# patrickltobing/shallow-wavenet

Measured on AMD Instinct MI355X. Metric: decoded samples/sec (22.05 kHz Laplacian AR decode, whole job), higher is better.
Workload: dtype f32

## Files before the change

include/swn_hip.h:

```cpp
#ifndef SWN_HIP_H
#define SWN_HIP_H

#include <stddef.h>
#include <stdint.h>

#ifdef __cplusplus
extern "C" {
#endif

#define SWN_ABI_VERSION 3

#define SWN_PRECISION_FP32 0
#define SWN_PRECISION_BF16 1

#define SWN_KIND_LAPLACE 0
#define SWN_KIND_SOFTMAX 1

#define SWN_OK            0
#define SWN_E_BADDESC    -1
#define SWN_E_BADARG     -2
#define SWN_E_LAUNCH     -3
#define SWN_E_UNSUPPORTED -4
#define SWN_E_NODEVICE   -5

// ... 47 lines not shown
    int32_t n_new;
    int32_t f0, f1;
    int32_t flags;
    int32_t reserved[2];
} swn_frontend_pool_entry;
#define SWN_FRONTEND_POOL_MAX_ENTRIES 64
#define SWN_FRONTEND_FINAL 1
size_t swn_frontend_pool_work_floats(const swn_net_desc* d, const swn_frontend_pool_entry* entries_host, int n_entries);
int    swn_frontend_pool(const swn_net_desc* d, const float* packed_dev, const swn_frontend_pool_entry* entries_host,
                         int n_entries, float* work_dev, void* stream);

#define SWN_POOL_MAX_MODELS 16
size_t swn_frontend_pool_models_work_floats(const swn_net_desc* d, const swn_frontend_pool_entry* entries_host,
                                            const int32_t* model_of_entry_host, int n_entries, int n_models);
int    swn_frontend_pool_models(const swn_net_desc* d, const float* const* models_host, int n_models,
                                const int32_t* model_of_entry_host, const swn_frontend_pool_entry* entries_host,
                                int n_entries, float* work_dev, void* stream);

typedef struct swn_decode_io {
    const float* noise_dev;
    const void*  forced_dev;
    const void*  seed_dev;
    float*       noise_out_dev;
    uint64_t     rng_seed;
    uint32_t     rng_utt0;
    uint32_t     reserved;
    const uint32_t* rng_utt_ids_dev;
} swn_decode_io;
size_t swn_decode_state_floats(const swn_net_desc* d, int batch);
int    swn_decode(const swn_net_desc* d, const float* packed_dev, const float* cond_dev,
                  int batch, int n_frames, int n_steps, const swn_decode_io* io,
                  float* state_dev, void* out_dev, float* heads_dev,
                  int variant, void* stream);

#define SWN_CHUNK_BEGIN 1
int    swn_decode_resolve_variant(const swn_net_desc* d, int batch, int variant);
size_t swn_decode_session_floats(const swn_net_desc* d, int batch, int variant);
int    swn_decode_chunk(const swn_net_desc* d, const float* packed_dev, const float* cond_dev, int batch, int n_frames,
                        int step0, int n_steps, int flags, const swn_decode_io* io, float* session_dev,
                        void* out_dev, float* heads_dev, int variant, void* stream);

typedef struct swn_decode_pool_entry {
    const float* cond_dev;
    int32_t n_frames;
    int32_t slot;
    int32_t step0;
    int32_t n_steps;
    int32_t flags;
    int32_t reserved;
} swn_decode_pool_entry;
#define SWN_DECODE_POOL_MAX_ENTRIES 64
int    swn_decode_pool_chunk(const swn_net_desc* d, const float* packed_dev, int capacity,
                             const swn_decode_pool_entry* entries_host, int n_entries,
                             const swn_decode_io* io, float* session_dev,
                             void* out_dev, float* heads_dev, int variant, void* stream);
int    swn_decode_pool_chunk_models(const swn_net_desc* d, const float* const* models_host, int n_models,
                                    const int32_t* model_of_entry_host, int capacity,
                                    const swn_decode_pool_entry* entries_host, int n_entries,
                                    const swn_decode_io* io, float* session_dev,
                                    void* out_dev, float* heads_dev, int variant, void* stream);

size_t swn_decode_w16_bytes(const swn_net_desc* d);
int    swn_pack_decode_w16(const swn_net_desc* d, const float* packed_dev, void* w16_dev, void* stream);
int    swn_decode_w16(const swn_net_desc* d, const float* packed_dev, const float* cond_dev,
                      int batch, int n_frames, int n_steps, const swn_decode_io* io,
                      float* state_dev, void* out_dev, float* heads_dev, int variant, const void* w16_dev, void* stream);
// ... 291 lines not shown
```

shallow_wavenet_amd/_lib.py:

```python
from __future__ import annotations

import ctypes
import os
import subprocess
import threading
from ctypes import POINTER, c_char_p, c_float, c_int, c_int32, c_int64, c_size_t, c_void_p

from .config import NetConfig

_HERE = os.path.dirname(os.path.abspath(__file__))
LIB_PATH = os.environ.get("SWN_HIP_LIB", os.path.join(_HERE, "libswn_hip.so"))
CSRC = os.path.join(_HERE, "csrc")

_lock = threading.Lock()
_lib = None


class NetDesc(ctypes.Structure):
    _fields_ = [(n, c_int32) for n in (
        "kind", "n_aux", "hid_chn", "skip_chn", "aux_kernel_size", "aux_dilation_size",
        "dilation_depth", "dilation_repeat", "kernel_size", "upsampling_factor", "seg", "lpc",
        "n_quantize", "wav_conv_flag", "audio_in_flag", "aux_conv2d_flag")]


# ... 84 lines not shown
                   aux_kernel_size=cfg.aux_kernel_size, aux_dilation_size=cfg.aux_dilation_size,
                   dilation_depth=cfg.dilation_depth, dilation_repeat=cfg.dilation_repeat,
                   kernel_size=cfg.kernel_size, upsampling_factor=cfg.upsampling_factor,
                   seg=1 if soft else cfg.seg, lpc=0 if soft else cfg.lpc,
                   n_quantize=cfg.n_quantize if soft else 0,
                   wav_conv_flag=int(cfg.wav_conv_flag), audio_in_flag=int(cfg.audio_in_flag and soft),
                   aux_conv2d_flag=int(cfg.aux_conv2d_flag and not soft))


SIGNATURES = {
    "swn_abi_version": (c_int, []),
    "swn_strerror": (c_char_p, [c_int]),
    "swn_last_error_detail": (c_char_p, []),
    "swn_device_count": (c_int, []),
    "swn_receptive_field": (c_int, [POINTER(NetDesc)]),
    "swn_num_tensors": (c_int, [POINTER(NetDesc)]),
    "swn_packed_floats": (c_size_t, [POINTER(NetDesc)]),
    "swn_layout_offsets": (c_int, [POINTER(NetDesc), POINTER(c_size_t), c_int]),
    "swn_pack_params": (c_int, [POINTER(NetDesc), POINTER(c_void_p), c_int, c_void_p, c_size_t]),
    "swn_pack_params_device": (c_int, [POINTER(NetDesc), POINTER(c_void_p), c_int, c_void_p, c_size_t, c_void_p]),
    "swn_frontend_conv_lds_bytes": (c_size_t, [POINTER(NetDesc), c_int]),
    "swn_frontend_work_floats": (c_size_t, [POINTER(NetDesc), c_int, c_int]),
    "swn_cond_floats": (c_size_t, [POINTER(NetDesc), c_int, c_int]),
    "swn_frontend": (c_int, [POINTER(NetDesc), c_void_p, c_void_p, c_int, c_int, c_void_p, c_void_p, c_void_p]),
    "swn_frontend_pool_work_floats": (c_size_t, [POINTER(NetDesc), POINTER(FrontendPoolEntry), c_int]),
    "swn_frontend_pool": (c_int, [POINTER(NetDesc), c_void_p, POINTER(FrontendPoolEntry), c_int, c_void_p, c_void_p]),
    "swn_frontend_pool_models_work_floats": (c_size_t, [POINTER(NetDesc), POINTER(FrontendPoolEntry), POINTER(c_int32), c_int,
                                                        c_int]),
    "swn_frontend_pool_models": (c_int, [POINTER(NetDesc), POINTER(c_void_p), c_int, POINTER(c_int32),
                                         POINTER(FrontendPoolEntry), c_int, c_void_p, c_void_p]),
    "swn_decode_state_floats": (c_size_t, [POINTER(NetDesc), c_int]),
    "swn_decode": (c_int, [POINTER(NetDesc), c_void_p, c_void_p, c_int, c_int, c_int, POINTER(DecodeIO),
                           c_void_p, c_void_p, c_void_p, c_int, c_void_p]),
    "swn_decode_resolve_variant": (c_int, [POINTER(NetDesc), c_int, c_int]),
    "swn_decode_session_floats": (c_size_t, [POINTER(NetDesc), c_int, c_int]),
    "swn_decode_chunk": (c_int, [POINTER(NetDesc), c_void_p, c_void_p, c_int, c_int, c_int, c_int, c_int, POINTER(DecodeIO),
                                 c_void_p, c_void_p, c_void_p, c_int, c_void_p]),
    "swn_decode_pool_chunk": (c_int, [POINTER(NetDesc), c_void_p, c_int, POINTER(DecodePoolEntry), c_int, POINTER(DecodeIO),
                                      c_void_p, c_void_p, c_void_p, c_int, c_void_p]),
    "swn_decode_pool_chunk_models": (c_int, [POINTER(NetDesc), POINTER(c_void_p), c_int, POINTER(c_int32), c_int,
                                             POINTER(DecodePoolEntry), c_int, POINTER(DecodeIO), c_void_p, c_void_p, c_void_p,
                                             c_int, c_void_p]),
    "swn_decode_pool_wide_table_bytes": (c_size_t, [c_int]),
    "swn_decode_pool_chunk_wide": (c_int, [POINTER(NetDesc), POINTER(c_void_p), c_int, POINTER(c_int32), c_int,
                                           POINTER(DecodePoolEntry), c_int, POINTER(DecodeIO), c_void_p, c_void_p, c_void_p,
                                           c_int, POINTER(c_void_p), c_int, c_void_p, c_void_p]),
    "swn_e4m3_table": (c_int, [c_void_p, c_float, c_void_p]),
    "swn_decode_stepped_prologue_iterations": (c_int, [POINTER(NetDesc)]),
    "swn_decode_pool_stepped_chunk": (c_int, [POINTER(NetDesc), c_void_p, c_int, POINTER(DecodeSteppedPoolEntry), c_int,
                                              POINTER(DecodeIO), c_void_p, c_void_p, c_void_p, c_void_p]),
    "swn_decode_stepped_pool_plan": (c_int, [POINTER(c_int32), POINTER(c_int32), c_int, c_int, c_int, POINTER(c_int32),
                                             POINTER(c_int32)]),
    "swn_decode_pool_stepped_chunk_models": (c_int, [POINTER(NetDesc), POINTER(c_void_p), c_int, POINTER(c_int32), c_int,
                                                     POINTER(DecodeSteppedPoolEntry), c_int, POINTER(DecodeIO), c_void_p,
                                                     c_void_p, c_void_p, c_void_p]),
    "swn_decode_stepped_prologue_work_floats": (c_size_t, [POINTER(NetDesc), c_int]),
    "swn_decode_stepped_prologue": (c_int, [POINTER(NetDesc), c_void_p, POINTER(c_void_p), c_int, POINTER(c_int32), c_int,
                                            POINTER(DecodeSteppedPrologueEntry), c_int, POINTER(DecodeIO), c_void_p, c_void_p,
                                            c_void_p]),
    "swn_postfilter_state_doubles": (c_size_t, [c_int, c_int, c_int]),
    "swn_postfilter_chunk": (c_int, [c_int, ctypes.c_double, c_int, c_void_p, c_int, c_void_p, c_void_p, c_void_p, c_int,
                                     POINTER(PostfilterEntry), c_int, c_void_p]),
    "swn_forward_work_floats": (c_size_t, [POINTER(NetDesc), c_int, c_int]),
    "swn_forward": (c_int, [POINTER(NetDesc), c_void_p, c_void_p, c_void_p, c_int, c_int, c_void_p,
                            c_void_p, c_void_p, c_void_p]),
    "swn_bf16_weight_bytes": (c_size_t, [POINTER(NetDesc)]),
# ... 150 lines not shown
```

shallow_wavenet_amd/csrc/swn_decode_bl6w.hip:

```cpp
#include <type_traits>
#include "swn_decode_bl6_common.hpp"
#include "swn_decode_internal.hpp"

#ifndef SWN_RES_SLICE
#define SWN_RES_SLICE 0
#endif
#ifndef SWN_ROTATE
#define SWN_ROTATE 1
#endif
#ifndef SWN_HANDOFF
#define SWN_HANDOFF 0
#endif
#ifndef SWN_OLDER2_MERGED
#define SWN_OLDER2_MERGED 1
#endif
#ifndef SWN_EARLY_ROWS
#define SWN_EARLY_ROWS 1
#endif
#ifndef SWN_LEAD
#define SWN_LEAD 1
#endif
#ifndef SWN_RINGX
#define SWN_RINGX 1
#endif
#ifdef SWN_STAMP
#define SWN_TDEF_PARAM , unsigned long long& tdef
#define SWN_TDEF_ARG(k) , td[k]
#else
#define SWN_TDEF_PARAM
#define SWN_TDEF_ARG(k)
#endif

namespace {

using namespace swn_bl6;

constexpr int NG = 256;
constexpr int S = 128;
constexpr int O1 = 128;

template <int LPC_, bool EXT_>
struct Tw {
    static constexpr int LPC = LPC_;
    static constexpr bool EXT = EXT_;
    using Ext = Tw<LPC_, true>;
    static constexpr bool NEWFORM = !EXT_ && LPC_ == 0;
    static constexpr int LEAD = NEWFORM ? SWN_LEAD : 0;
    static constexpr bool RINGX = NEWFORM && SWN_RINGX;
    static constexpr int NO = 2 + LPC_;
    static constexpr int WN = cmax(1, LPC_) + 1;
    static constexpr int ring_len(int l) { return pow2ceil((1 << l) + 1); }
    static constexpr int ring_off(int l) { int o = 0; for (int i = 0; i < l; ++i) o += ring_len(i) * H; return o; }
    static constexpr int PF = L * 2 * H;
    static constexpr int NZC = 64, NZB = 4;
    static constexpr int o_ring = 0;
    static constexpr int o_hcat = o_ring + ring_off(L);
    static constexpr int o_gp = o_hcat + L * H;
    static constexpr int o_bx = o_gp + 2 * PF;
    static constexpr int o_bd = o_bx + L * 2 * H;
    static constexpr int o_old = o_bd + L * 2 * H;
    static constexpr int o_wup = o_old + 2 * L * 2 * H;
    static constexpr int o_skip = o_wup + 256;
    static constexpr int o_p2 = o_skip + S;
    static constexpr int o_tnz = o_p2 + 4 * NO;
    static constexpr int o_cz = o_tnz + r4(NZB * NZC);
    static constexpr int o_w2 = o_cz + 5 * H;
    static constexpr int o_bias = o_w2 + NO * S + r4(NO);
    static constexpr int o_w1 = o_bias + S + O1;
    static constexpr int o_wl = o_w1 + 8 * O1 * 16;
    static constexpr int o_h0w = o_wl + 8 * NG * 4;
    static constexpr int o_ho = o_h0w + 3 * H;
    static constexpr int HO = 4, NHO = 128;
    static constexpr int o_end = o_ho + (NEWFORM && (SWN_HANDOFF & 1) && SWN_ROTATE ? NHO * HO : 0);
    static constexpr size_t lds_bytes = (size_t)o_end * sizeof(float);
    static constexpr int sess_old = ring_off(L);
    static constexpr int sess_win = sess_old + 2 * L * 2 * H;
    static constexpr int sess_floats = sess_win + r4(WN);
};

__device__ __forceinline__ float sum_quads(float v) {
    v += dpp_f<0x124>(v);
    v += dpp_f<0x128>(v);
    float w = v;
    asm("s_nop 1\n\tv_permlane16_swap_b32 %0, %1" : "+v"(v), "+v"(w));
    v += w;
    w = v;
    asm("s_nop 1\n\tv_permlane32_swap_b32 %0, %1" : "+v"(v), "+v"(w));
    return v + w;
}
__device__ __forceinline__ float quad_sum_by_parity(float own, float other) {
    float s = own + dpp_f<0xB1>(other);
    s += dpp_f<0x4E>(s);
    return s;
}
struct NoWork { __device__ __forceinline__ void operator()() const {} };
template <class T, int LAYER, int NQ = 2, class BEHIND = NoWork>
__device__ __forceinline__ void layer_a(float* lds, const float (&w)[2][16], const int q, const float wj, const int pb, const int po,
                                        const int ta, const float* xr, BEHIND&& behind = NoWork{}) {
    constexpr bool ROT = !std::is_same<typename std::decay<BEHIND>::type, NoWork>::value;
    const int o = ta >> 2, p = ta & 3, pr = p & 1;
    const float e_old = lds[T::o_old + po + LAYER * 2 * H + pr * H + o];
    const float g_gp = lds[T::o_gp + pb + LAYER * 2 * H + pr * H + o], g_bx = lds[T::o_bx + LAYER * 2 * H + pr * H + o];
    const float e_hp = xr[o];
    static_assert(NQ >= 0 && NQ <= 4, "early quads");
    float4 xq[4];
    if constexpr (ROT) {
#pragma unroll
        for (int m = 0; m < NQ; ++m) xq[m] = *reinterpret_cast<const float4*>(xr + 16 * p + 4 * m);
        __builtin_amdgcn_sched_barrier(0);
        behind();
        __builtin_amdgcn_sched_barrier(0);
    }
    const float e_gx = fmaf(wj, g_gp, g_bx);
    float az = 0.f, ac = 0.f;
#pragma unroll
    for (int m = 0; m < 4; ++m) {
        float4 x;
        if (ROT && m < NQ) x = xq[m];
        else x = *reinterpret_cast<const float4*>(xr + 16 * p + 4 * m);
        az = fmaf(w[0][4 * m], x.x, az); ac = fmaf(w[1][4 * m], x.x, ac);
        az = fmaf(w[0][4 * m + 1], x.y, az); ac = fmaf(w[1][4 * m + 1], x.y, ac);
        az = fmaf(w[0][4 * m + 2], x.z, az); ac = fmaf(w[1][4 * m + 2], x.z, ac);
        az = fmaf(w[0][4 * m + 3], x.w, az); ac = fmaf(w[1][4 * m + 3], x.w, ac);
    }
    const float sq = quad_sum_by_parity(pr ? ac : az, pr ? az : ac);
    __builtin_amdgcn_sched_barrier(0);
    if (p < 2) {
        const float sa = sq + e_old;
        const float v = e_gx * sa;
#ifdef SWN_DIAG_PLAINEXP
        const float e = __builtin_amdgcn_exp2f((p == 0 ? -v : -2.f * fminf(fabsf(v), 64.f)) * 1.44269504f);
        const float r = __builtin_amdgcn_rcpf(1.f + e);
#else
        const float e = exp_c(p == 0 ? -v : -2.f * fminf(fabsf(v), 64.f));
        const float r = rcp_c(1.f + e);
#endif
        const float res = p == 0 ? r : copysignf((1.f - e) * r, v);
        const float c = dpp_f<0xF5>(res);
        if (p == 0) {
            const float hn = (1.f - res) * c + res * e_hp;
            if (LAYER + 1 < L) {
                constexpr int R2 = T::ring_len(LAYER + 1 < L ? LAYER + 1 : LAYER);
                lds[T::o_ring + T::ring_off(LAYER + 1 < L ? LAYER + 1 : LAYER) + (q & (R2 - 1)) * H + o] = hn;
            }
            if (!T::RINGX || LAYER + 1 >= L) lds[T::o_hcat + LAYER * H + o] = hn;
        }
    }
    __builtin_amdgcn_sched_barrier(0);
}

template <class T, int LAYER, int MB = 4>
__device__ __forceinline__ void older_sum(const float* lds, const float (&w)[2][16], const int qn, const int tb, float& az, float& ac) {
    constexpr int dil = 1 << LAYER;
    constexpr int R = T::ring_len(LAYER);
    const int p = tb & 3;
    const float* ring = lds + T::o_ring + T::ring_off(LAYER);
    az = 0.f; ac = 0.f;
#pragma unroll
    for (int m = 0; m < 4; ++m) {
        const float4 x = *reinterpret_cast<const float4*>(ring + ((qn - dil) & (R - 1)) * H + 16 * p + 4 * m);
        float4 w0, w1;
        if (LAYER < L - 1) {
            w0 = make_float4(w[0][4 * m], w[0][4 * m + 1], w[0][4 * m + 2], w[0][4 * m + 3]);
            w1 = make_float4(w[1][4 * m], w[1][4 * m + 1], w[1][4 * m + 2], w[1][4 * m + 3]);
        } else {
            w0 = *reinterpret_cast<const float4*>(lds + T::o_wl + (m * NG + tb) * 4);
            w1 = *reinterpret_cast<const float4*>(lds + T::o_wl + ((4 + m) * NG + tb) * 4);
        }
        az = fmaf(w0.x, x.x, az); ac = fmaf(w1.x, x.x, ac);
        az = fmaf(w0.y, x.y, az); ac = fmaf(w1.y, x.y, ac);
        az = fmaf(w0.z, x.z, az); ac = fmaf(w1.z, x.z, ac);
        az = fmaf(w0.w, x.w, az); ac = fmaf(w1.w, x.w, ac);
        if (MB < 4 && m % MB == MB - 1) __builtin_amdgcn_sched_barrier(0);
    }
    az = sum4(az); ac = sum4(ac);
}
template <class T, int LAYER>
__device__ __forceinline__ void older_store(float* lds, const int qn, const int tb, const float az, const float ac) {
    const int o = tb >> 2, p = tb & 3, pr = p & 1;
    lds[T::o_old + (qn & 1) * (L * 2 * H) + LAYER * 2 * H + pr * H + o] = (p == 0 ? az : ac) + lds[T::o_bd + LAYER * 2 * H + pr * H + o];
}
// ... 144 lines not shown
        }
        __builtin_amdgcn_sched_barrier(0);
    }
    asm volatile("" : "+v"(sacc[0]), "+v"(sacc[1]));
}
template <class T>
__device__ __forceinline__ void skip_last_b(float* lds, const float4 (&wsl)[8], const float (&sacc)[2], const int tb) {
    const int r = tb >> 2, hp = tb & 3;
    float part[2][4];
#pragma unroll
    for (int mm = 0; mm < 4; ++mm) {
        const float4 x = *reinterpret_cast<const float4*>(lds + T::o_hcat + (L - 1) * H + 16 * mm + 4 * hp);
#pragma unroll
        for (int ps = 0; ps < 2; ++ps) {
            const float4 w = wsl[ps * 4 + mm];
            part[ps][mm] = fmaf(w.w, x.w, fmaf(w.z, x.z, fmaf(w.y, x.y, w.x * x.x)));
        }
    }
    float s[2];
#pragma unroll
    for (int ps = 0; ps < 2; ++ps) s[ps] = sacc[ps] + ((part[ps][0] + part[ps][1]) + (part[ps][2] + part[ps][3]));
    const float t0 = s[0] + dpp_f<0xB1>(s[0]), t1 = s[1] + dpp_f<0xB1>(s[1]);
    const float v = (hp < 2 ? t0 : t1) + dpp_f<0x4E>(hp < 2 ? t1 : t0);
    if ((hp & 1) == 0) lds[T::o_skip + r + 32 * hp] = fmaxf(v, 0.f);
}

template <bool MOVE2> using OlderMergedT = typename std::conditional<MOVE2, Layers<2, 3, 4>, Layers<3, 4>>::type;
template <bool MOVE2> using OlderOut1T = typename std::conditional<MOVE2, Layers<0, 1>, Layers<0, 1, 2>>::type;
template <int E> struct Out1Split;
template <> struct Out1Split<2> { using Early = Layers<0, 1>; using Late = Layers<>; };
template <> struct Out1Split<1> { using Early = Layers<0>; using Late = Layers<1>; };
template <> struct Out1Split<0> { using Early = Layers<>; using Late = Layers<0, 1>; };

template <class T, bool GA, bool STREAM, bool POOL = false>
__device__ __forceinline__ void decode_body(const Bl6Args& a, float* lds) {
    constexpr bool EXT = T::EXT;
    static_assert(!STREAM || EXT, "streamed chunks run the extended mode");
    constexpr bool grpA = GA;
    const int tid = threadIdx.x, b = POOL ? 0 : blockIdx.x;
    __builtin_assume(GA ? tid < NG : tid >= NG);
    const int tg = tid & (NG - 1);
    const float* __restrict__ P = a.P;
    const int U = a.U;
    const int s0 = STREAM ? a.step0 : 0;
    const bool resume = STREAM && a.resume;
    const int fb0 = STREAM ? s0 / U : 0;

    for (int e = tid; e < T::o_end; e += NT) lds[e] = 0.f;
    __syncthreads();
    for (int e = tid; e < L * 2 * H; e += NT) {
        lds[T::o_bx + e] = P[a.y.bx + e];
        const float bd = P[a.y.bd + e];
        lds[T::o_bd + e] = bd;
        lds[T::o_old + e] = bd;
    }
    for (int e = tid; e < U; e += NT) lds[T::o_wup + e] = P[a.y.wup + e];
    for (int e = tid; e < H; e += NT) lds[T::o_cz + e] = P[a.y.cb + e];
    for (int e = tid; e < S; e += NT) lds[T::o_bias + e] = P[a.y.bsk + e];
    for (int e = tid; e < O1; e += NT) lds[T::o_bias + S + e] = P[a.y.b1 + e];
    for (int e = tid; e < 2 * H; e += NT) { lds[T::o_cz + H + e] = P[a.y.cv + e]; lds[T::o_cz + 3 * H + e] = P[a.y.cc + e]; }
    for (int e = tid; e < T::NO * S; e += NT) lds[T::o_w2 + e] = P[a.y.w2 + (size_t)(e / S) * r4(S) + (e % S)];
    for (int e = tid; e < T::NO; e += NT) lds[T::o_w2 + T::NO * S + e] = P[a.y.b2 + e];
    for (int e = tid; e < 8 * O1 * 16; e += NT) lds[T::o_w1 + e] = P[a.y.w12 + e];
    const __amdgpu_buffer_rsrc_t condr =
        make_rsrc(a.cond + (size_t)b * a.Tf * a.N, (unsigned)((size_t)a.Tf * a.N * sizeof(float)));
    auto load_frame = [&](int fr) {
        float* dst = lds + T::o_gp + (fr & 1) * T::PF;
#pragma unroll
        for (int it = 0; it < (T::PF / 4 + NT - 1) / NT; ++it) {
            const int e4 = it * NT + tid;
            if (e4 < T::PF / 4)
                *reinterpret_cast<float4*>(dst + 4 * e4) =
                    buf_ld4(condr, (unsigned)tid * 16u, (unsigned)(fr * a.N * 4 + it * NT * 16));
        }
    };
    for (int fr = fb0; fr < fb0 + 2 && fr < a.Tf; ++fr) load_frame(fr);
    constexpr int NWR = grpA ? L : L - 1;
    float wreg[NWR][2][16];
    {
        const int o = tg >> 2, p = tg & 3, k = grpA ? 1 : 0;
#pragma unroll
        for (int l = 0; l < L; ++l)
#pragma unroll
            for (int r = 0; r < 2; ++r) {
                const float4* src = reinterpret_cast<const float4*>(P + a.y.wd + (((size_t)l * 2 * H + o + r * H) * 2 + k) * H + 16 * p);
#pragma unroll
                for (int v = 0; v < 4; ++v) {
                    const float4 t = src[v];
                    if (l == L - 1 && !grpA) {
                        *reinterpret_cast<float4*>(lds + T::o_wl + ((r * 4 + v) * NG + tg) * 4) = t;
                    } else {
                        float (&wr)[16] = wreg[l < NWR ? l : 0][r];
                        wr[4 * v] = t.x; wr[4 * v + 1] = t.y; wr[4 * v + 2] = t.z; wr[4 * v + 3] = t.w;
                    }
                }
            }
    }
    __syncthreads();
    const float* sess_b = STREAM ? a.sess + (size_t)b * T::sess_floats : nullptr;
    int tcp = tid;
    asm volatile("" : "+v"(tcp));
    if (resume) {
        for (int e = tcp; e < T::ring_off(L); e += NT) lds[T::o_ring + e] = sess_b[e];
        for (int e = tcp; e < 2 * L * 2 * H; e += NT) lds[T::o_old + e] = sess_b[T::sess_old + e];
        __syncthreads();
    }

    int fb = fb0, tb0 = fb0 * U;
    const int n_pro = RF;
    auto cond_taps = [&](int q, float& wj, int& pb) {
        const int t0 = q - RF;
        const int tlo = t0 < 0 ? 0 : t0;
        if (tlo >= tb0 + U) {
            fb += 1; tb0 += U;
            if (fb + 1 < a.Tf) load_frame(fb + 1);
        }
        int rel = tlo - tb0;
        int fsel = fb;
// ... 71 lines not shown
                const float sg = (e > 0.f) ? 1.f : ((e < 0.f) ? -1.f : 0.f);
                lds[T::o_tnz + (c & (T::NZB - 1)) * T::NZC + k] = sg * log1pf(-2.f * fabsf(e));
            }
            if (!EXT) noise_load(c + 1);
        }
    };
    if (!EXT && NZG && tn >= 64 && tn < 128) noise_load(0);
    noise_chunk(0);
    noise_chunk(1);

    const __amdgpu_buffer_rsrc_t wsk2 = make_rsrc(P + a.y.wsk2, (unsigned)(L * S * 64 * sizeof(float)));
    constexpr bool NEWFORM = T::NEWFORM;
    constexpr int RES = (grpA || !NEWFORM) ? -1 : SWN_RES_SLICE;
    static_assert(RES == -1 || RES == 0 || RES == L - 1, "the first or the last slice");
    constexpr int LEADB = RES == 0 ? T::LEAD : 0;
    static_assert(LEADB == 0 || LEADB == 1 || LEADB == 2 || LEADB == 4, "one load, a quarter or a half of a slice");
    float4 wres[8];
    if constexpr (RES == 0) skip_issue_b<0>(wsk2, wres, tg, 0u);
    if constexpr (RES == L - 1) skip_issue_b<L - 1>(wsk2, wres, tg, 0u);

#ifdef SWN_STAMP
    unsigned long long tw[9] = {0, 0, 0, 0, 0, 0, 0, 0, 0}, tv[6] = {0, 0, 0, 0, 0, 0}, td[5] = {0, 0, 0, 0, 0}, tstep = 0, tlast = 0, tbeg = 0;
#define SWN_BAR(k) { tw[k] += __builtin_amdgcn_s_memtime() - tlast; lds_barrier(); tlast = __builtin_amdgcn_s_memtime(); }
#define SWN_WAIT_STAMP(k) { asm volatile("" :: "v"(wsl[0].x)); tv[k] += __builtin_amdgcn_s_memtime() - tlast; }
#define SWN_PRE(k) { tw[k] += __builtin_amdgcn_s_memtime() - tlast; asm volatile("s_waitcnt lgkmcnt(0)" ::: "memory"); }
#define SWN_BAR_KEEP(k, N) { lds_barrier_keep<N>(); tlast = __builtin_amdgcn_s_memtime(); }
#else
#define SWN_BAR(k) lds_barrier();
#define SWN_WAIT_STAMP(k)
#define SWN_PRE(k)
#define SWN_BAR_KEEP(k, N) lds_barrier_keep<N>();
#endif
#define SWN_PHASE_WORK(LAYER, GEN, X0)                                                                                \
    if constexpr (grpA) layer_a<T, LAYER>(lds, wreg[LAYER], q, wj, pb, po, tg,                                         \
                                          LAYER == 0 ? (X0) : lds + T::o_ring + T::ring_off(LAYER) +                   \
                                                                  (q & (T::ring_len(LAYER) - 1)) * H);                 \
    else {                                                                                                             \
        if (GEN) {    \
                      \
                      \
                      \
            if (LAYER == 0) { if (RES != 0) skip_issue_b<0>(wsk2, wsl, tg, step0); }                                   \
                      \
            else if (LAYER == 1 && RES == 0)                                                                           \
                skip_roll_b<T, 1, !NOSTREAM, LEADB, LEADB, true>(lds, wsk2, wres, wsl, sacc, tg, step0, q SWN_TDEF_ARG(0)); \
            else { SWN_WAIT_STAMP(LAYER > 0 ? LAYER - 1 : 0)                                                           \
                   skip_roll_b<T, (LAYER > 0 ? LAYER : 1), !(LAYER == L - 1 && RES == L - 1) && !NOSTREAM,             \
                               (LAYER >= 2 ? LEADB : 0), (LAYER < L - 1 ? LEADB : 0)>(lds, wsk2, wsl, wsl, sacc, tg, step0, q \
                                                                                      SWN_TDEF_ARG(LAYER > 0 ? LAYER - 1 : 0)); } \
            __builtin_amdgcn_sched_barrier(0);                                                                         \
        }                                                                                                              \
        if (!(GEN)) older_b<T, LAYER>(lds, wreg[LAYER < NWR ? LAYER : 0], q + 1, tg);                                  \
        else if (LAYER == 0) older_bn<T>(OlderMerged{}, lds, wreg, q + 1, tg);                                         \
        __builtin_amdgcn_sched_barrier(0);                                                                             \
    }
#define SWN_PHASE(LAYER, GEN, X0) SWN_PHASE_WORK(LAYER, GEN, X0) if (GEN) { SWN_BAR(LAYER) } else lds_barrier();

#pragma unroll 1
    for (int q = resume ? n_pro : 0; q < n_pro; ++q) {
        float wj; int pb;
        float4 wsl[8]; float sacc[2]; const unsigned step0 = 0;
        cond_taps(q, wj, pb);
        const int po = (q & 1) * (L * 2 * H);
        input_seed(q);
        lds_barrier();
        const float* x0 = lds + T::o_ring + (q & 1) * H;
        SWN_PHASE(0, false, x0) SWN_PHASE(1, false, x0) SWN_PHASE(2, false, x0) SWN_PHASE(3, false, x0)
        SWN_PHASE(4, false, x0) SWN_PHASE(5, false, x0)
        (void)wsl; (void)sacc; (void)step0;
    }

    int rel_c = s0 - fb0 * U;
    bool fill_c = false;
    float wj_c = 0.f;
    int pb_c = 0, po_c = 0, x0_c = 0;
    auto taps_ahead = [&](int qn) {
        wj_c = lds[T::o_wup + rel_c];
        pb_c = (fb & 1) * T::PF;
        po_c = (qn & 1) * (L * 2 * H);
        x0_c = h0_row(qn);
        asm volatile("" : "+s"(pb_c), "+s"(po_c), "+s"(x0_c));
    };
    auto frame_advance = [&]() {
        rel_c += 1;
        const bool cross = rel_c >= U;
        if (cross) { rel_c = 0; fb += 1; }
        fill_c = cross && fb + 1 < a.Tf;
    };
    if constexpr (grpA) taps_ahead(RF + s0);
    input_gen(x0_c);
#ifdef SWN_STAMP
    tlast = tbeg = __builtin_amdgcn_s_memtime();
#endif
    constexpr bool ROT = SWN_ROTATE && NEWFORM;
    constexpr int ROTQ = 2;
    float sv_p = 0.f, acc_p = 0.f;
    const __amdgpu_buffer_rsrc_t outr =
        make_rsrc(reinterpret_cast<float*>(a.out) + (size_t)b * a.n_steps, (unsigned)((size_t)a.n_steps * sizeof(float)));
    const __amdgpu_buffer_rsrc_t headr =
        make_rsrc(HEADS_ON && a.heads ? a.heads + (size_t)b * a.n_steps * T::NO : nullptr,
                  HEADS_ON && a.heads ? (unsigned)((size_t)a.n_steps * T::NO * sizeof(float)) : 0u);
    auto store_step = [&](const int ip) __attribute__((always_inline)) {
// ... 18 lines not shown
        }
    };
    auto load_frame_b = [&](int fr) {
        if (tg < T::PF / 4)
            *reinterpret_cast<float4*>(lds + T::o_gp + (fr & 1) * T::PF + 4 * tg) =
                buf_ld4(condr, (unsigned)tg * 16u, (unsigned)(fr * a.N * 4));
    };
    auto store_chunk_b = [&](const int c) __attribute__((always_inline)) {
        const int step = c * 64 + tg;
        if (tg < 64 && step < a.n_steps) {
            const float4 v = *reinterpret_cast<const float4*>(lds + T::o_ho + (step & (T::NHO - 1)) * T::HO);
            __builtin_amdgcn_raw_buffer_store_b32(__builtin_bit_cast(unsigned, v.z), outr, (unsigned)tg * 4u, (unsigned)c * 256u, 0);
            using u2 = unsigned __attribute__((ext_vector_type(2)));
            u2 h; h.x = __builtin_bit_cast(unsigned, v.x); h.y = __builtin_bit_cast(unsigned, v.y);
            __builtin_amdgcn_raw_buffer_store_b64(h, headr, (unsigned)tg * 8u, (unsigned)c * 512u, 0);
        }
    };
    auto gen_step = [&](const int i) __attribute__((always_inline)) {
        const int q = RF + s0 + i;
        const float wj = wj_c;
        const int pb = pb_c, po = po_c;
        if constexpr (grpA && !ROT) {
            if (fill_c) load_frame(fb + 1);
        }
        auto behind0 = [&]() __attribute__((always_inline)) {
            if constexpr (NOSIDE) return;
            if constexpr (!HO_NZ) { if ((i & (T::NZC - 1)) == 0) noise_chunk((i >> 6) + 2); }
            if constexpr (!HO_RF) { if (fill_c) load_frame(fb + 1); }
            if constexpr (HO_ST) { if (i > 0) ho_write(i - 1); }
            else { if (i > 0) store_step(i - 1); }
        };
        float4 wsl[8];
        float sacc[2] = {0.f, 0.f};
        if constexpr (!grpA) {
            const float bs0 = lds[T::o_bias + (tg >> 2)], bs1 = lds[T::o_bias + (tg >> 2) + 64];
            if ((tg & 3) == 0) { sacc[0] = bs0; sacc[1] = bs1; }
        }
        unsigned step0 = 0;
        asm volatile("" : "+s"(step0));
        const float* x0 = lds + x0_c;
#ifdef SWN_DIAG_NOSIDE_B
        constexpr bool SIDE_B = false;
#else
        constexpr bool SIDE_B = HOFF && !grpA && !NOSIDE;
#endif
        if constexpr (SIDE_B) {
            __builtin_amdgcn_sched_barrier(0);
            if constexpr (HO_NZ) { if ((i & (T::NZC - 1)) == 0) noise_chunk((i >> 6) + 2); }
            if constexpr (HO_RF) { if (fill_c) load_frame_b(fb + 1); }
            if constexpr (HO_ST) { if ((i & 63) == 1 && i > 1) store_chunk_b((i >> 6) - 1); }
            __builtin_amdgcn_sched_barrier(0);
        }
        if constexpr (NOSTREAM && !grpA) {
#pragma unroll
            for (int k = 0; k < 8; ++k) asm volatile("" : "=v"(wsl[k].x), "=v"(wsl[k].y), "=v"(wsl[k].z), "=v"(wsl[k].w));
        }
        if constexpr (grpA && ROT) {
            layer_a<T, 0, ROTQ>(lds, wreg[0], q, wj, pb, po, tg, x0, behind0);
            SWN_BAR(0)
        } else {
            SWN_PHASE(0, true, x0)
        }
        SWN_PHASE(1, true, x0) SWN_PHASE(2, true, x0) SWN_PHASE(3, true, x0)
        SWN_PHASE(4, true, x0)
        constexpr bool EARLY5 = T::LPC == 0;
        float4 xl[2], wl[2][2];
        SWN_PHASE_WORK(5, true, x0)
        if constexpr (grpA && EARLY5) {
            SWN_PRE(5)
            lds_fence_compiler();
            __builtin_amdgcn_sched_barrier(0);
            older_last_rows<T>(lds, q + 1, tg + (int)step0, xl, wl);
            __builtin_amdgcn_sched_barrier(0);
            SWN_BAR_KEEP(5, 6)
        } else {
            SWN_BAR(5)
        }
        constexpr bool ROLL1 = T::LPC == 0;
        using Split = Out1Split<MOVE2 ? NEARLY : 2>;
        float4 xo[cmax(NEARLY, 1)][4];
        float4 w1e[2][2];
        if constexpr (!grpA) {
            if constexpr (RES == L - 1) skip_last_b<T>(lds, wres, sacc, tg);
            else { SWN_WAIT_STAMP(5) skip_last_b<T>(lds, wsl, sacc, tg); }
            SWN_PRE(6)
            lds_fence_compiler();
            __builtin_amdgcn_sched_barrier(0);
            if constexpr (!MOVE2) {
                older_rows_n<T>(OlderOut1{}, lds, q + 1, tg, xo);
                __builtin_amdgcn_sched_barrier(0);
                SWN_BAR_KEEP(6, 12)
// ... 57 lines not shown
                for (int mm = 0; mm < 8; ++mm) {
                    fma8(mm, X(mm), W(mm, 0), W(mm, 1));
                    if ((mm & 3) == 3) __builtin_amdgcn_sched_barrier(0);
                }
            }
            const float v = sum4(a0 + a1), u = sum4(b0 + b1);
            if constexpr (ROLL1) {
                const float o1a = fmaxf(v + e_b1[0], 0.f), o1b = fmaxf(u + e_b1[1], 0.f);
                const float pz = sum_quads(fmaf(e_w2[1], o1b, fmaf(e_w2[0], o1a, tg < 4 ? e_b2 : 0.f)));
                if ((tg & 63) < 4 && hp < T::NO) lds[T::o_p2 + 4 * hp + wv] = pz;
            } else {
                const float o1a = fmaxf(v + lds[T::o_bias + S + hr], 0.f), o1b = fmaxf(u + lds[T::o_bias + S + hr + 64], 0.f);
#pragma unroll
                for (int j = 0; j < (T::NO + 3) / 4; ++j) {
                    const int k = hp + 4 * j, kc = k < T::NO ? k : T::NO - 1;
                    const float* w2 = lds + T::o_w2 + kc * S;
                    const float b2 = lds[T::o_w2 + T::NO * S + kc];
                    const float pz = sum_quads(fmaf(w2[hr + 64], o1b, fmaf(w2[hr], o1a, tg < 4 ? b2 : 0.f)));
                    if ((tg & 63) < 4 && k < T::NO) lds[T::o_p2 + 4 * k + wv] = pz;
                }
            }
        } else if constexpr (!MOVE2) {
            older_bn_x<T>(OlderOut1{}, lds, wreg, xo, q + 1, tg);
        } else {
            if constexpr (NEARLY > 0) older_bn_x<T>(typename Split::Early{}, lds, wreg, xo, q + 1, tg);
            if constexpr (NEARLY < NOUT1) older_bn<T>(typename Split::Late{}, lds, wreg, q + 1, tg);
        }
        SWN_BAR(7)
        if constexpr (grpA) {
            const int ln = tg & 63;
            float tz = 0.f;
            if constexpr (!EXT) tz = lds[T::o_tnz + (i & (T::NZB * T::NZC - 1))];
            float fv = 0.f;
            if (a.forced) fv = reinterpret_cast<const float*>(a.forced)[(size_t)b * a.n_steps + i];
            const float4 pz = *reinterpret_cast<const float4*>(lds + T::o_p2 + 4 * (ln < T::NO ? ln : T::NO - 1));
            __builtin_amdgcn_sched_barrier(0);
            frame_advance();
            taps_ahead(q + 1);
            __builtin_amdgcn_sched_barrier(0);
            const float acc = (pz.x + pz.y) + (pz.z + pz.w);
            float o2[T::NO];
#pragma unroll
            for (int k = 0; k < T::NO; ++k) o2[k] = __builtin_bit_cast(float, __builtin_amdgcn_readlane(__builtin_bit_cast(int, acc), k));
            float sv;
            {
#pragma clang fp contract(off)
                const float mu = o2[0];
                const float bsc = sigm(o2[1]);
                float lpv = 0.f;
#pragma unroll
                for (int k = 0; k < T::LPC; ++k) lpv += o2[2 + T::LPC - 1 - k] * win[T::WN - T::LPC + k];
                const float t = bsc * (EXT ? lds[T::o_tnz + ((i >> 6) & (T::NZB - 1)) * T::NZC + (i & (T::NZC - 1))] : tz);
                sv = (T::LPC > 0) ? (lpv + mu) - t : mu - t;
                sv = fminf(fmaxf(sv, -1.f), 1.f);
                float fd = a.forced ? fv : sv;
                asm volatile("" : "+v"(fd));
#pragma unroll
                for (int k = 0; k + 1 < T::WN; ++k) win[k] = win[k + 1];
                win[T::WN - 1] = fd;
            }
            if (i + 1 < a.n_steps) input_gen(x0_c);
            __builtin_amdgcn_sched_barrier(0);
            if constexpr (ROT) { sv_p = sv; acc_p = acc; }
            else {
                if (tid == 0) reinterpret_cast<float*>(a.out)[(size_t)b * a.n_steps + (size_t)i] = sv;
                if (HEADS_ON && a.heads && wv == 0 && ln < T::NO) a.heads[((size_t)b * a.n_steps + i) * T::NO + ln] = acc;
            }
        }
        if constexpr (HO_RF && !grpA) frame_advance();
#ifdef SWN_STAMP
        if constexpr (grpA) tw[8] += __builtin_amdgcn_s_memtime() - tlast;
#endif
    };
    if constexpr (ROT) {
#pragma unroll 1
        for (int i = 0; i < a.n_steps; ++i) gen_step(i);
        if constexpr (HO_ST) {
            if constexpr (grpA) { if (a.n_steps > 0) ho_write(a.n_steps - 1); }
            lds_barrier();
            if constexpr (!grpA) {
                for (int c = a.n_steps >= 66 ? ((a.n_steps - 66) >> 6) + 1 : 0; c * 64 < a.n_steps; ++c) store_chunk_b(c);
            }
        } else if (a.n_steps > 0) store_step(a.n_steps - 1);
    } else {
#pragma unroll 1
        for (int i0 = 0; i0 < a.n_steps; i0 += T::NZC) {
            noise_chunk((i0 >> 6) + 2);
            const int iend = i0 + T::NZC < a.n_steps ? i0 + T::NZC : a.n_steps;
#pragma unroll 1
            for (int i = i0; i < iend; ++i) gen_step(i);
        }
    }
#ifdef SWN_STAMP
    { const unsigned long long tn = __builtin_amdgcn_s_memtime(); tw[0] += tn - tlast; tstep = tn - tbeg; }
#endif
    if constexpr (STREAM) {
        __syncthreads();
        float* so = a.sess + (size_t)b * T::sess_floats;
        tcp = tid;
        asm volatile("" : "+v"(tcp));
        for (int e = tcp; e < T::ring_off(L); e += NT) so[e] = lds[T::o_ring + e];
        for (int e = tcp; e < 2 * L * 2 * H; e += NT) so[T::sess_old + e] = lds[T::o_old + e];
        if (tid == 0) {
#pragma unroll
            for (int k = 0; k < T::WN; ++k) so[T::sess_win + k] = win[k];
        }
    }
#undef SWN_PHASE
#undef SWN_PHASE_WORK
#undef SWN_BAR
#undef SWN_WAIT_STAMP
#undef SWN_PRE
#undef SWN_BAR_KEEP
#ifdef SWN_STAMP
    if ((tid == 0 || tid == 64 || tid == NG) && b == 0 && a.heads) {
        float* h = a.heads + (tid == 0 ? 0 : tid == 64 ? 30 : 10);
        for (int k = 0; k < 9; ++k) h[k] = (float)((double)tw[k] / (double)a.n_steps);
        if (tid == 0) h[9] = (float)((double)tstep / (double)a.n_steps);
        else if (tid == NG) {
            for (int k = 0; k < 6; ++k) h[10 + k] = (float)((double)tv[k] / (double)a.n_steps);
            for (int k = 0; k < 5; ++k) h[34 + k] = (float)((double)td[k] / (double)a.n_steps);
        }
    }
#endif
}

template <class T, bool STREAM = false>
__global__ __launch_bounds__(NT) void decode_bl6w_kernel(const Bl6Args a) {
    extern __shared__ __attribute__((aligned(16))) float lds[];
    if (threadIdx.x < NG) decode_body<T, true, STREAM>(a, lds);
    else decode_body<T, false, STREAM>(a, lds);
}

template <class T, bool MODELS = false>
__global__ __launch_bounds__(NT) void decode_bl6w_pool_kernel(
    const typename std::conditional<MODELS, Bl6PoolModelsArgs, Bl6PoolArgs>::type p) {
    extern __shared__ __attribute__((aligned(16))) float lds[];
    static_assert(T::EXT, "pools run the extended mode");
    Bl6Args a = p.c;
    if constexpr (MODELS) a.P = swn_pool_model(p.m);
    if (!swn_pool_entry_args(a, p.t, 1, 1, T::NO)) return;
    a.sess += (size_t)swn_pool_slot(p.t) * T::sess_floats;
    if (threadIdx.x < NG) decode_body<T, true, true, true>(a, lds);
    else decode_body<T, false, true, true>(a, lds);
}

template <class T>
__global__ __launch_bounds__(NT) void decode_bl6w_pool_wide_kernel(const Bl6PoolWideArgs p) {
    extern __shared__ __attribute__((aligned(16))) float lds[];
    static_assert(T::EXT, "pools run the extended mode");
    Bl6Args a = p.c;
    const SwnPoolWideRow row = swn_pool_wide_row(p.rows);
    a.P = row.model;
    if (!swn_pool_entry_args(a, row.e, 1, 1, T::NO)) return;
    a.sess += (size_t)row.e.slot * T::sess_floats;
    if (threadIdx.x < NG) decode_body<T, true, true, true>(a, lds);
    else decode_body<T, false, true, true>(a, lds);
}

bool bl6w_applies(const SwnGeom& g) {
    return g.bl6 && g.U <= 256 && g.U >= 2 && !g.audio_in && g.kind == SWN_KIND_LAPLACE && g.S == 128 && g.O1 == 128 &&
           g.seg == 1 && (g.lpc == 0 || g.lpc == 4);
}

// ... 8 lines not shown

int swn_decode_bl6w_run(const SwnDecodeCall& c) {
    const hipStream_t st = c.hip_stream;
    if (c.wide) {
        Bl6PoolWideArgs p;
        fill_args(p.c, c);
        p.rows = c.wide;
        return with_tw(c.g, [&](auto tw) {
            using T = typename decltype(tw)::Ext;
            return launch_kernel(decode_bl6w_pool_wide_kernel<T>, T::lds_bytes, c.batch, p, st, "swn_decode_pool_chunk_wide(bl6w)");
        });
    }
    if (c.pool) {
        Bl6PoolModelsArgs p;
        fill_args(p.c, c);
        p.t = *c.pool;
        if (c.models) p.m = *c.models;
        return with_tw(c.g, [&](auto tw) {
            using T = typename decltype(tw)::Ext;
            if (c.models)
                return launch_kernel(decode_bl6w_pool_kernel<T, true>, T::lds_bytes, c.batch, p, st, "swn_decode_pool_chunk_models(bl6w)");
            const Bl6PoolArgs& p1 = p;
            return launch_kernel(decode_bl6w_pool_kernel<T>, T::lds_bytes, c.batch, p1, st, "swn_decode_pool_chunk(bl6w)");
        });
    }
    Bl6Args a;
    fill_args(a, c);
    return with_tw(c.g, [&](auto t) {
        using T = decltype(t);
        using X = typename T::Ext;
        static_assert(T::lds_bytes <= 160 * 1024 && X::lds_bytes <= 160 * 1024, "LDS budget");
        if (c.stream) return launch_kernel(decode_bl6w_kernel<X, true>, X::lds_bytes, a.B, a, st, "swn_decode(bl6w)");
        if (wants_ext(a)) return launch_kernel(decode_bl6w_kernel<X>, X::lds_bytes, a.B, a, st, "swn_decode(bl6w)");
        return launch_kernel(decode_bl6w_kernel<T>, T::lds_bytes, a.B, a, st, "swn_decode(bl6w)");
    });
}

size_t swn_decode_bl6w_session_floats(const SwnGeom& g) {
    int n = 0;
    with_tw(g, [&](auto t) { n = decltype(t)::sess_floats; return SWN_OK; });
    return (size_t)n;
}
```

Before: 411,800.

## Swap weight rows per parity and flatten the gated-activation epilogue in bl6w decode

```diff
diff --git a/include/swn_hip.h b/include/swn_hip.h
--- a/include/swn_hip.h
+++ b/include/swn_hip.h
@@ -103,6 +103,7 @@
                   int batch, int n_frames, int n_steps, const swn_decode_io* io,
                   float* state_dev, void* out_dev, float* heads_dev,
                   int variant, void* stream);
+size_t swn_decode_bl6w_lds_bytes(const swn_net_desc* d, int extended);
 
 #define SWN_CHUNK_BEGIN 1
 int    swn_decode_resolve_variant(const swn_net_desc* d, int batch, int variant);
diff --git a/shallow_wavenet_amd/_lib.py b/shallow_wavenet_amd/_lib.py
--- a/shallow_wavenet_amd/_lib.py
+++ b/shallow_wavenet_amd/_lib.py
@@ -140,6 +140,7 @@
     "swn_decode_state_floats": (c_size_t, [POINTER(NetDesc), c_int]),
     "swn_decode": (c_int, [POINTER(NetDesc), c_void_p, c_void_p, c_int, c_int, c_int, POINTER(DecodeIO),
                            c_void_p, c_void_p, c_void_p, c_int, c_void_p]),
+    "swn_decode_bl6w_lds_bytes": (c_size_t, [POINTER(NetDesc), c_int]),
     "swn_decode_resolve_variant": (c_int, [POINTER(NetDesc), c_int, c_int]),
     "swn_decode_session_floats": (c_size_t, [POINTER(NetDesc), c_int, c_int]),
     "swn_decode_chunk": (c_int, [POINTER(NetDesc), c_void_p, c_void_p, c_int, c_int, c_int, c_int, c_int, POINTER(DecodeIO),
diff --git a/shallow_wavenet_amd/csrc/swn_decode_bl6w.hip b/shallow_wavenet_amd/csrc/swn_decode_bl6w.hip
--- a/shallow_wavenet_amd/csrc/swn_decode_bl6w.hip
+++ b/shallow_wavenet_amd/csrc/swn_decode_bl6w.hip
@@ -22,6 +22,18 @@
 #endif
 #ifndef SWN_RINGX
 #define SWN_RINGX 1
+#endif
+#ifndef SWN_CARRY_HP
+#define SWN_CARRY_HP 0
+#endif
+#ifndef SWN_SWAP_ROWS
+#define SWN_SWAP_ROWS 1
+#endif
+#ifndef SWN_FLAT_EPILOGUE
+#define SWN_FLAT_EPILOGUE 1
+#endif
+#ifndef SWN_PLAIN_TAIL
+#define SWN_PLAIN_TAIL 0
 #endif
 #ifdef SWN_STAMP
 #define SWN_TDEF_PARAM , unsigned long long& tdef
@@ -71,12 +83,26 @@
     static constexpr int o_h0w = o_wl + 8 * NG * 4;
     static constexpr int o_ho = o_h0w + 3 * H;
     static constexpr int HO = 4, NHO = 128;
-    static constexpr int o_end = o_ho + (NEWFORM && (SWN_HANDOFF & 1) && SWN_ROTATE ? NHO * HO : 0);
+    static constexpr bool CARRY_HP = NEWFORM && SWN_CARRY_HP;
+    static constexpr bool SWAP_ROWS = NEWFORM && SWN_SWAP_ROWS;
+    static constexpr bool FLAT_EPI = NEWFORM && SWN_FLAT_EPILOGUE;
+    static constexpr bool PLAIN_TAIL = NEWFORM && SWN_PLAIN_TAIL;
+    static constexpr int o_dump = o_ho + (NEWFORM && (SWN_HANDOFF & 1) && SWN_ROTATE ? NHO * HO : 0);
+    static constexpr int o_end = o_dump + (FLAT_EPI ? NG : 0);
     static constexpr size_t lds_bytes = (size_t)o_end * sizeof(float);
+    static_assert(o_dump == o_wl + 8 * NG * 4 + 3 * H + (o_dump - o_ho) && (o_dump - o_ho == 0 || o_dump - o_ho == NHO * HO),
+                  "the carve ends with group B's last-layer half, the three h0 copies and the hand-off ring");
+    static_assert(o_end - o_dump == (FLAT_EPI ? NG : 0) && (!FLAT_EPI || o_dump + (NG - 1) == o_end - 1),
+                  "one dump word per thread of group A, the last one the carve's last float");
+    static_assert(o_dump % 4 == 0 && (size_t)o_end * sizeof(float) <= 160 * 1024, "16-byte carve, 160 KB of LDS");
     static constexpr int sess_old = ring_off(L);
     static constexpr int sess_win = sess_old + 2 * L * 2 * H;
     static constexpr int sess_floats = sess_win + r4(WN);
 };
+static_assert((SWN_HANDOFF & 1) || Tw<0, false>::o_dump == 39308, "classic lpc 0 carve");
+static_assert((SWN_HANDOFF & 1) || !SWN_FLAT_EPILOGUE || Tw<0, false>::o_end == 39564, "classic lpc 0 carve with the dump words");
+static_assert(Tw<0, true>::o_end == Tw<0, true>::o_dump && Tw<4, false>::o_end == Tw<4, false>::o_dump &&
+              Tw<4, true>::o_end == Tw<4, true>::o_dump, "the other kernels keep the parent's carve");
 
 __device__ __forceinline__ float sum_quads(float v) {
     v += dpp_f<0x124>(v);
@@ -95,13 +121,13 @@
 }
 struct NoWork { __device__ __forceinline__ void operator()() const {} };
 template <class T, int LAYER, int NQ = 2, class BEHIND = NoWork>
-__device__ __forceinline__ void layer_a(float* lds, const float (&w)[2][16], const int q, const float wj, const int pb, const int po,
-                                        const int ta, const float* xr, BEHIND&& behind = NoWork{}) {
+__device__ __forceinline__ float layer_a(float* lds, const float (&w)[2][16], const int q, const float wj, const int pb, const int po,
+                                         const int ta, const float* xr, const float hp_in, BEHIND&& behind = NoWork{}) {
     constexpr bool ROT = !std::is_same<typename std::decay<BEHIND>::type, NoWork>::value;
     const int o = ta >> 2, p = ta & 3, pr = p & 1;
     const float e_old = lds[T::o_old + po + LAYER * 2 * H + pr * H + o];
     const float g_gp = lds[T::o_gp + pb + LAYER * 2 * H + pr * H + o], g_bx = lds[T::o_bx + LAYER * 2 * H + pr * H + o];
-    const float e_hp = xr[o];
+    const float e_hp = (T::CARRY_HP && LAYER >= 1) ? hp_in : xr[o];
     static_assert(NQ >= 0 && NQ <= 4, "early quads");
     float4 xq[4];
     if constexpr (ROT) {
@@ -123,8 +149,24 @@
         az = fmaf(w[0][4 * m + 2], x.z, az); ac = fmaf(w[1][4 * m + 2], x.z, ac);
         az = fmaf(w[0][4 * m + 3], x.w, az); ac = fmaf(w[1][4 * m + 3], x.w, ac);
     }
-    const float sq = quad_sum_by_parity(pr ? ac : az, pr ? az : ac);
+    const float sq = T::SWAP_ROWS ? quad_sum_by_parity(az, ac) : quad_sum_by_parity(pr ? ac : az, pr ? az : ac);
     __builtin_amdgcn_sched_barrier(0);
+    float hn = 0.f;
+    if constexpr (T::FLAT_EPI) {
+        const float sa = sq + e_old;
+        const float v = e_gx * sa;
+        const float e = exp_c(pr == 0 ? -v : -2.f * fminf(fabsf(v), 64.f));
+        const float r = rcp_c(1.f + e);
+        const float res = pr == 0 ? r : copysignf((1.f - e) * r, v);
+        const float c = dpp_f<0xF5>(res);
+        hn = (1.f - res) * c + res * e_hp;
+        constexpr int R2 = T::ring_len(LAYER + 1 < L ? LAYER + 1 : LAYER);
+        const int dst = LAYER + 1 < L ? T::o_ring + T::ring_off(LAYER + 1 < L ? LAYER + 1 : LAYER) + (q & (R2 - 1)) * H + o
+                                      : T::o_hcat + LAYER * H + o;
+        static_assert(T::RINGX || !T::FLAT_EPI, "one hand-off store per layer");
+        float* const own = lds + T::o_dump + ta;
+        *(p == 0 ? lds + dst : own) = hn;
+    } else
     if (p < 2) {
         const float sa = sq + e_old;
         const float v = e_gx * sa;
@@ -138,7 +180,7 @@
         const float res = p == 0 ? r : copysignf((1.f - e) * r, v);
         const float c = dpp_f<0xF5>(res);
         if (p == 0) {
-            const float hn = (1.f - res) * c + res * e_hp;
+            hn = (1.f - res) * c + res * e_hp;
             if (LAYER + 1 < L) {
                 constexpr int R2 = T::ring_len(LAYER + 1 < L ? LAYER + 1 : LAYER);
                 lds[T::o_ring + T::ring_off(LAYER + 1 < L ? LAYER + 1 : LAYER) + (q & (R2 - 1)) * H + o] = hn;
@@ -147,6 +189,7 @@
         }
     }
     __builtin_amdgcn_sched_barrier(0);
+    return hn;
 }
 
 template <class T, int LAYER, int MB = 4>
@@ -357,8 +400,9 @@
 template <> struct Out1Split<1> { using Early = Layers<0>; using Late = Layers<1>; };
 template <> struct Out1Split<0> { using Early = Layers<>; using Late = Layers<0, 1>; };
 
-template <class T, bool GA, bool STREAM, bool POOL = false>
+template <class T, bool GA, bool STREAM, bool POOL = false, bool PLAIN = false>
 __device__ __forceinline__ void decode_body(const Bl6Args& a, float* lds) {
+    static_assert(!PLAIN || (T::PLAIN_TAIL && !STREAM), "the one-shot classic lpc 0 kernel");
     constexpr bool EXT = T::EXT;
     static_assert(!STREAM || EXT, "streamed chunks run the extended mode");
     constexpr bool grpA = GA;
@@ -408,7 +452,8 @@
         for (int l = 0; l < L; ++l)
 #pragma unroll
             for (int r = 0; r < 2; ++r) {
-                const float4* src = reinterpret_cast<const float4*>(P + a.y.wd + (((size_t)l * 2 * H + o + r * H) * 2 + k) * H + 16 * p);
+                const int rs = (grpA && T::SWAP_ROWS) ? r ^ (p & 1) : r;
+                const float4* src = reinterpret_cast<const float4*>(P + a.y.wd + (((size_t)l * 2 * H + o + rs * H) * 2 + k) * H + 16 * p);
 #pragma unroll
                 for (int v = 0; v < 4; ++v) {
                     const float4 t = src[v];
@@ -546,9 +591,9 @@
 #define SWN_BAR_KEEP(k, N) lds_barrier_keep<N>();
 #endif
 #define SWN_PHASE_WORK(LAYER, GEN, X0)                                                                                \
-    if constexpr (grpA) layer_a<T, LAYER>(lds, wreg[LAYER], q, wj, pb, po, tg,                                         \
-                                          LAYER == 0 ? (X0) : lds + T::o_ring + T::ring_off(LAYER) +                   \
-                                                                  (q & (T::ring_len(LAYER) - 1)) * H);                 \
+    if constexpr (grpA) hcar = layer_a<T, LAYER>(lds, wreg[LAYER], q, wj, pb, po, tg,                                  \
+                                                 LAYER == 0 ? (X0) : lds + T::o_ring + T::ring_off(LAYER) +            \
+                                                                         (q & (T::ring_len(LAYER) - 1)) * H, hcar);    \
     else {                                                                                                             \
         if (GEN) {    \
                       \
@@ -574,6 +619,7 @@
     for (int q = resume ? n_pro : 0; q < n_pro; ++q) {
         float wj; int pb;
         float4 wsl[8]; float sacc[2]; const unsigned step0 = 0;
+        float hcar = 0.f;
         cond_taps(q, wj, pb);
         const int po = (q & 1) * (L * 2 * H);
         input_seed(q);
@@ -581,7 +627,7 @@
         const float* x0 = lds + T::o_ring + (q & 1) * H;
         SWN_PHASE(0, false, x0) SWN_PHASE(1, false, x0) SWN_PHASE(2, false, x0) SWN_PHASE(3, false, x0)
         SWN_PHASE(4, false, x0) SWN_PHASE(5, false, x0)
-        (void)wsl; (void)sacc; (void)step0;
+        (void)wsl; (void)sacc; (void)step0; (void)hcar;
     }
 
     int rel_c = s0 - fb0 * U;
@@ -666,6 +712,7 @@
         };
         float4 wsl[8];
         float sacc[2] = {0.f, 0.f};
+        float hcar = 0.f;
         if constexpr (!grpA) {
             const float bs0 = lds[T::o_bias + (tg >> 2)], bs1 = lds[T::o_bias + (tg >> 2) + 64];
             if ((tg & 3) == 0) { sacc[0] = bs0; sacc[1] = bs1; }
@@ -690,7 +737,7 @@
             for (int k = 0; k < 8; ++k) asm volatile("" : "=v"(wsl[k].x), "=v"(wsl[k].y), "=v"(wsl[k].z), "=v"(wsl[k].w));
         }
         if constexpr (grpA && ROT) {
-            layer_a<T, 0, ROTQ>(lds, wreg[0], q, wj, pb, po, tg, x0, behind0);
+            hcar = layer_a<T, 0, ROTQ>(lds, wreg[0], q, wj, pb, po, tg, x0, hcar, behind0);
             SWN_BAR(0)
         } else {
             SWN_PHASE(0, true, x0)
@@ -814,7 +861,8 @@
             float tz = 0.f;
             if constexpr (!EXT) tz = lds[T::o_tnz + (i & (T::NZB * T::NZC - 1))];
             float fv = 0.f;
-            if (a.forced) fv = reinterpret_cast<const float*>(a.forced)[(size_t)b * a.n_steps + i];
+            const bool forced_on = !PLAIN && a.forced;
+            if (forced_on) fv = reinterpret_cast<const float*>(a.forced)[(size_t)b * a.n_steps + i];
             const float4 pz = *reinterpret_cast<const float4*>(lds + T::o_p2 + 4 * (ln < T::NO ? ln : T::NO - 1));
             __builtin_amdgcn_sched_barrier(0);
             frame_advance();
@@ -835,13 +883,13 @@
                 const float t = bsc * (EXT ? lds[T::o_tnz + ((i >> 6) & (T::NZB - 1)) * T::NZC + (i & (T::NZC - 1))] : tz);
                 sv = (T::LPC > 0) ? (lpv + mu) - t : mu - t;
                 sv = fminf(fmaxf(sv, -1.f), 1.f);
-                float fd = a.forced ? fv : sv;
+                float fd = forced_on ? fv : sv;
                 asm volatile("" : "+v"(fd));
 #pragma unroll
                 for (int k = 0; k + 1 < T::WN; ++k) win[k] = win[k + 1];
                 win[T::WN - 1] = fd;
             }
-            if (i + 1 < a.n_steps) input_gen(x0_c);
+            if (PLAIN || i + 1 < a.n_steps) input_gen(x0_c);
             __builtin_amdgcn_sched_barrier(0);
             if constexpr (ROT) { sv_p = sv; acc_p = acc; }
             else {
@@ -907,11 +955,11 @@
 #endif
 }
 
-template <class T, bool STREAM = false>
+template <class T, bool STREAM = false, bool PLAIN = false>
 __global__ __launch_bounds__(NT) void decode_bl6w_kernel(const Bl6Args a) {
     extern __shared__ __attribute__((aligned(16))) float lds[];
-    if (threadIdx.x < NG) decode_body<T, true, STREAM>(a, lds);
-    else decode_body<T, false, STREAM>(a, lds);
+    if (threadIdx.x < NG) decode_body<T, true, STREAM, false, PLAIN>(a, lds);
+    else decode_body<T, false, STREAM, false, PLAIN>(a, lds);
 }
 
 template <class T, bool MODELS = false>
@@ -986,8 +1034,26 @@
         static_assert(T::lds_bytes <= 160 * 1024 && X::lds_bytes <= 160 * 1024, "LDS budget");
         if (c.stream) return launch_kernel(decode_bl6w_kernel<X, true>, X::lds_bytes, a.B, a, st, "swn_decode(bl6w)");
         if (wants_ext(a)) return launch_kernel(decode_bl6w_kernel<X>, X::lds_bytes, a.B, a, st, "swn_decode(bl6w)");
+        if constexpr (T::PLAIN_TAIL) {
+            if (!a.forced) return launch_kernel(decode_bl6w_kernel<T, false, true>, T::lds_bytes, a.B, a, st, "swn_decode(bl6w)");
+        }
         return launch_kernel(decode_bl6w_kernel<T>, T::lds_bytes, a.B, a, st, "swn_decode(bl6w)");
     });
+}
+
+size_t swn_decode_bl6w_lds(const SwnGeom& g, bool extended) {
+    size_t n = 0;
+    with_tw(g, [&](auto t) {
+        using T = decltype(t);
+        n = extended ? T::Ext::lds_bytes : T::lds_bytes;
+        return SWN_OK;
+    });
+    return n;
+}
+extern "C" size_t swn_decode_bl6w_lds_bytes(const swn_net_desc* d, int extended) {
+    SwnGeom g;
+    if (swn_make_geom(d, &g) < 0) return 0;
+    return swn_decode_bl6w_lds(g, extended != 0);
 }
 
 size_t swn_decode_bl6w_session_floats(const SwnGeom& g) {
```

Result: faster. 419,600 (median of 6 runs) (+1.9%).
